# gargatik/Seamless-Through-Breaking-Rethinking-Image-Stitching-for-Optimal-Alignment

Hardware: AMD Instinct MI355X
Metric: stitched image-pairs/s at 512x512 (higher is better)
Workload: dtype f32 (decoder contractions, PatchEmbed's third conv and the C = 128 block tails: exact 3xbf16 split of both operands, 6 products on the bf16 matrix cores, fp32 accumulate -- error vs fp64 0.83x the fp32 MFMA chain's; everything else fp32); 1 GPU; UDIS-D-shaped 512x512 pairs, batch=1, FlowHomoAdpater.forward(type=test_eval); launch=hipGraph replay, pairs_in_flight=3

## Files before the change

include/stitch_gfx950.h:

```cpp
#ifndef STITCH_GFX950_H
#define STITCH_GFX950_H
#include <stdint.h>
#ifdef __cplusplus
extern "C" {
#endif

typedef struct st_gemm_desc {
    const float* a;
    const float* w;
    float* c;
    const float* bias;
    const float* aux0;
    const float* aux1;
    const float* aux2;
    const float* scale_ptr;
    int32_t M, N, K;
    int32_t H, W, Cin, ldx;
    int32_t kh, kw, sh, sw, ph, pw, Ho, Wo;
    int32_t ldw, ldc, ld_aux0, ld_aux1, ld_aux2;
    int32_t aux0_row_div, aux0_row_mod;
    int32_t act;
    int32_t epi;
    float alpha;
    int32_t batch;
// ... 66 lines not shown
    const float* w1;
    const float* b1;
    const float* w2;
    const float* b2;
    const float* res;
    int32_t lda, ldo, ld_res, M, hidden, ln;
    float ln_eps;
    int32_t reserved;
    const float* wp;
    const float* bp;
    const float* res0;
    int32_t ld_res0, reserved1;
} st_mlp_desc;
int st_mlp128(const st_mlp_desc* desc, void* stream);
int st_abi_mlp_desc_size(void);
int st_mlp128_split3_image_bytes(int32_t hidden, int32_t with_proj, int64_t* bytes);
int st_mlp128_split3_pack(const float* w1, const float* b1, const float* w2, const float* wp, const float* bp, int32_t hidden, void* image,
                          int64_t image_bytes, void* stream);
int st_mlp128_split3(const st_mlp_desc* desc, const void* image, int64_t image_bytes, void* stream);
int st_rowlin128_split3_image_bytes(int32_t N, int64_t* bytes);
int st_rowlin128_split3_pack(const float* w, const float* b, int32_t N, void* image, int64_t image_bytes, void* stream);
int st_rowlin128_split3(const float* a, int32_t lda, float* out, int32_t ldo, int32_t M, int32_t N, int32_t ln, float ln_eps, const void* image,
                        int64_t image_bytes, const float* aux, int32_t ld_aux, int32_t row_div, void* stream);

int st_corr_volume(const float* f1, const float* f2, float* vol, int32_t B, int32_t N1, int32_t N2,
                   int32_t C, void* stream);
int st_corr_volume_both(const float* f1, const float* f2, float* vol12, float* vol21, int32_t B, int32_t N, int32_t C,
                        void* stream);
int st_corr_volume_both_plan(int32_t B, int32_t N, int32_t C, int32_t aligned16);

int st_layernorm(const float* x, int32_t ldx, const float* w, const float* b, float* out, int32_t ldo,
                 int32_t rows, int32_t C, float eps, void* stream);
int st_softmax_rows(float* x, int32_t ld, int32_t rows, int32_t C, void* stream);
int st_l2norm_rows(const float* x, float* out, int32_t rows, int32_t C, void* stream);
int st_maxpool_nhwc(const float* x, float* out, int32_t B, int32_t H, int32_t W, int32_t C, int32_t k,
                    int32_t s, int32_t p, void* stream);
int st_dwconv3x3_residual(const float* x, const float* w, const float* bias, float* out, int32_t B,
                          int32_t H, int32_t W, int32_t C, void* stream);
int st_sine_pe(float* out, int32_t ld, int32_t rows, int32_t dim, const float* coords, int32_t ldc,
               int32_t Wg, int32_t ws, int32_t period, float cscale, float coff, int32_t accumulate,
               void* stream);
int st_attention_small(const float* q, int64_t q_bs, int64_t q_ts, const float* k, int64_t k_bs, int64_t k_ts,
                       const float* v, int64_t v_bs, int64_t v_ts, float* out, int64_t o_bs, int64_t o_ts,
                       int32_t B, int32_t heads, int32_t Nq, int32_t Nk, int32_t D, float scale, void* stream);
int st_attention_kvlds(const float* q, int64_t q_bs, int64_t q_ts, const float* k, int64_t k_bs, int64_t k_ts,
                       const float* v, int64_t v_bs, int64_t v_ts, float* out, int64_t o_bs, int64_t o_ts,
// ... 292 lines not shown
```

seamless-through-breaking-rethinking-image-stitching-for-optimal-alignment_amd/build.py:

```python
from __future__ import annotations

import os
import subprocess
import sys
from concurrent.futures import ThreadPoolExecutor

HERE = os.path.dirname(os.path.abspath(__file__))
CSRC = os.path.join(HERE, "csrc")
OUT = os.path.join(HERE, "libstitch_gfx950.so")
HIPCC = os.environ.get("HIPCC", "/opt/rocm/bin/hipcc")
SOURCES = {"gemm.hip": [], "gemm_split3.hip": [], "gemm_rows.hip": [], "nn.hip": [], "flowops.hip": [], "geom.hip": ["-ffp-contract=off"],
           "metrics.hip": ["-ffp-contract=off"], "operators.hip": [], "composition.hip": ["-ffp-contract=off"], "tps_pipeline.hip": ["-ffp-contract=off"], "patchembed.hip": [],
           "inpaint.hip": ["-ffp-contract=off"], "tps_other.hip": ["-ffp-contract=off"],
           "transref.hip": ["-ffp-contract=off"], "flow_splat.hip": ["-ffp-contract=off"], "jpeg.hip": [], "jpeg_dec.hip": [],
           "multiband.hip": ["-ffp-contract=off"], "exposure.hip": ["-ffp-contract=off"], "seam.hip": [], "seam_gc.hip": [], "crop.hip": [], "patchmatch.hip": [],
           "features.hip": ["-ffp-contract=off"], "dense_flow.hip": ["-ffp-contract=off"], "features_ms.hip": ["-ffp-contract=off"]}
COMMON = ["--offload-arch=gfx950", "-O3", "-std=c++17", "-fPIC", "-Wno-unused-result"]
COMMON += ["-Xclang", "-target-feature", "-Xclang", "-packed-fp32-ops"]
if os.environ.get("ST_EXACT_TRANSCENDENTALS", "0") == "1":
    COMMON.append("-DST_EXACT_TRANSCENDENTALS")


def compile_cmd(src, out, extra=()):
    return [HIPCC] + COMMON + SOURCES[src] + list(extra) + [os.path.join(CSRC, src), "-o", out]


def _stale(target, deps):
    if not os.path.exists(target):
        return True
    t = os.path.getmtime(target)
    return any(os.path.getmtime(d) > t for d in deps)


def build(force=False, verbose=False):
    hdrs = [os.path.join(CSRC, "common.h"), os.path.join(CSRC, "gemm_common.h"), os.path.join(CSRC, "gemm_split3.h"), os.path.join(CSRC, "mlp_split3.h"), os.path.join(CSRC, "tps_solve.h"), os.path.join(CSRC, "jpeg_dec_core.h"), os.path.join(CSRC, "jpeg_tables.h"), os.path.join(CSRC, "jpeg_huff_core.h"), os.path.join(CSRC, "jpeg_scan.h"), os.path.join(CSRC, "jpeg_rst_core.h"), os.path.join(CSRC, "features_common.h"), os.path.join(HERE, "..", "include", "stitch_gfx950.h")]
    objs, jobs = [], []
    os.makedirs(os.path.join(CSRC, "_obj"), exist_ok=True)
    for src in SOURCES:
        s = os.path.join(CSRC, src)
        o = os.path.join(CSRC, "_obj", src.replace(".hip", ".o"))
        objs.append(o)
        if force or _stale(o, [s] + hdrs):
            jobs.append(compile_cmd(src, o, ["-c"]))
    if jobs:
        def run(cmd):
            if verbose:
                print(" ".join(cmd), flush=True)
            r = subprocess.run(cmd, stderr=subprocess.PIPE, text=True)
            err = "".join(l for l in r.stderr.splitlines(True) if "'-packed-fp32-ops' is not a recognized feature for this target" not in l)
            if err:
                sys.stderr.write(err)
            if r.returncode:
                raise subprocess.CalledProcessError(r.returncode, cmd)
        with ThreadPoolExecutor(max_workers=4) as ex:
            list(ex.map(run, jobs))
    if jobs or _stale(OUT, objs):
        subprocess.check_call([HIPCC, "--offload-arch=gfx950", "-shared", "-fPIC", "-o", OUT] + objs)
    return OUT
# ... 5 lines not shown
```

seamless-through-breaking-rethinking-image-stitching-for-optimal-alignment_amd/csrc/gemm_rows.hip:

```cpp
#include "gemm_common.h"

static bool row_launch_begin(st_gemm_desc& od, int kernel, int tile, void* stream, const float* a, int lda, float* c, int ldc, const void* w, int M, int N,
                             int split3) {
    bool obs = st_observer_installed();
    if (obs) {
        od = Gemm(a, lda, (const float*)w, 128, c, ldc, M, N, 128).d;
        od.split3 = split3;
        obs = st_observe(&od, stream, 0);
    }
    st_plan_set(kernel, tile, 1, 1);
    return obs;
}

#define RC_NW 4
__global__ __launch_bounds__(256, 2) void rowchain128_kernel(const st_chain_desc d) {
    constexpr int NJ = 16, NW = RC_NW;
    extern __shared__ __attribute__((aligned(1024))) float smem[];
    float* ring = smem;
    const int tid = threadIdx.x, lane = tid & 63, wave = __builtin_amdgcn_readfirstlane(tid >> 6);
    const int li = lane & 31, lh = lane >> 5;
    const int nblk = (d.M + 31) >> 5;
    const int G = (int)gridDim.x;
    const int blk0 = (int)blockIdx.x * NW;
    const int rounds = blk0 < nblk ? (nblk - blk0 + G * NW - 1) / (G * NW) : 0;
// ... 456 lines not shown
}
extern "C" int st_rowlin128_split3(const float* a, int32_t lda, float* out, int32_t ldo, int32_t M, int32_t N, int32_t ln, float ln_eps, const void* image,
                                   int64_t image_bytes, const float* aux, int32_t ld_aux, int32_t row_div, void* stream) {
    if (aux && (ld_aux < N || (ld_aux & 3) || row_div < 1 || ((uintptr_t)aux & 15) || aux == out)) return ST_EINVAL;
    if (!a || !out || !image || M <= 0 || N < 32 || N > 4096 || (N & 31) || lda < 128 || ldo < N || (lda & 3) || (ldo & 3) || a == out) return ST_EINVAL;
    if ((((uintptr_t)a | (uintptr_t)out | (uintptr_t)image) & 15) || (int64_t)M * (lda > ldo ? lda : ldo) >= ((int64_t)1 << 40)) return ST_EINVAL;
    const int64_t need = (int64_t)(N / 32) * LS3_STAGE_B;
    if (image_bytes < need) return ST_EINVAL;
    const int nblk = (M + 31) / 32;
    int G = (nblk + 3) / 4;
    if (G > 512) G = 512;
    const size_t lds = (size_t)3 * LS3_STAGE_B;
    auto kern = aux ? rowlin128_split3_kernel<true> : rowlin128_split3_kernel<false>;
    (void)hipFuncSetAttribute((const void*)kern, hipFuncAttributeMaxDynamicSharedMemorySize, (int)lds);
    st_gemm_desc od;
    const bool obs = row_launch_begin(od, 10, 40, stream, a, lda, out, ldo, image, M, N, 1);
    hipLaunchKernelGGL(kern, dim3(G), dim3(256), lds, (hipStream_t)stream, a, (int)lda, out, (int)ldo, (int)M, (int)N, (int)ln, ln_eps,
                       (const unsigned char*)image, (unsigned)need, aux, (int)ld_aux, (int)(row_div > 0 ? row_div : 1));
    if (obs) st_observe(&od, stream, 1);
    ST_CHECK_LAUNCH();
    return ST_OK;
}

extern "C" int st_pe_tail_split3_image_bytes(int64_t* bytes) {
    if (!bytes) return ST_EINVAL;
    *bytes = PT3_IMAGE_B;
    return ST_OK;
}
extern "C" int st_pe_tail_split3_pack(const float* w1, int32_t ld1, const float* w2, void* image, int64_t image_bytes, void* stream) {
    if (!w1 || !w2 || !image || ld1 < 64 || ((uintptr_t)image & 15) || image_bytes < PT3_IMAGE_B) return ST_EINVAL;
    hipLaunchKernelGGL(pe_tail_split3_pack_kernel, dim3(3, 4), dim3(256), 0, (hipStream_t)stream, w1, (int)ld1, w2, (unsigned char*)image);
    ST_CHECK_LAUNCH();
    return ST_OK;
}
extern "C" int st_pe_tail_split3(const float* x, const float* tab, int32_t P, const void* image, int64_t image_bytes, const float* b2, const float* gamma,
                                 const float* beta, float eps, float* out, int32_t R, void* stream) {
    if (!x || !tab || !image || !b2 || !gamma || !beta || !out || R <= 0 || P <= 0 || image_bytes < PT3_IMAGE_B || x == out) return ST_EINVAL;
    if ((((uintptr_t)x | (uintptr_t)tab | (uintptr_t)image | (uintptr_t)out) & 15) || (int64_t)R * 128 >= ((int64_t)1 << 40)) return ST_EINVAL;
    const int nblk = (R + 31) / 32;
    int G = (nblk + 3) / 4;
    if (G > 256) G = 256;
    bool tabinv = false;
    for (int g = G; g >= (G > 8 ? G - G / 8 : 1); --g)
        if (((long)g * 128) % P == 0) { G = g; tabinv = true; break; }
    const size_t lds = (size_t)PT3_IMAGE_B + PT3_VEC_B;
    auto kern = tabinv ? pe_tail_split3_kernel<true> : pe_tail_split3_kernel<false>;
// ... 9 lines not shown
```

seamless-through-breaking-rethinking-image-stitching-for-optimal-alignment_amd/csrc/mlp_split3.h:

```cpp
#pragma once
#include "gemm_common.h"

#define MS3_W1_B 24576
#define MS3_W2_B 24576
#define MS3_BIAS_B 1024
#define MS3_STAGE_B (MS3_W1_B + MS3_W2_B + MS3_BIAS_B)
#define MS3_PIECES (MS3_STAGE_B / 1024)

typedef __bf16 bf16x2_t __attribute__((ext_vector_type(2)));
typedef float f32x2_t __attribute__((ext_vector_type(2)));

__device__ __forceinline__ unsigned ms3_pk(float a, float b) {
    const f32x2_t v = {a, b};
    return __builtin_bit_cast(unsigned, __builtin_convertvector(v, bf16x2_t));
}
__device__ __forceinline__ void ms3_split_pair(float x0, float x1, unsigned& h, unsigned& m, unsigned& l) {
    h = ms3_pk(x0, x1);
    const float r0 = x0 - __uint_as_float(h << 16), r1 = x1 - __uint_as_float(h & 0xffff0000u);
    m = ms3_pk(r0, r1);
    l = ms3_pk(r0 - __uint_as_float(m << 16), r1 - __uint_as_float(m & 0xffff0000u));
}

__global__ __launch_bounds__(256) void mlp_split3_pack_kernel(const float* __restrict__ w1, const float* __restrict__ b1, const float* __restrict__ w2,
                                                              const float* __restrict__ wp, const float* __restrict__ bp, int hidden,
// ... 445 lines not shown
                    MS3_SIX(acc, f, xp[0][ks], xp[1][ks], xp[2][ks])
#pragma unroll
                    for (int p = 0; p < 3; ++p) f[p] = fn[p];
                    __builtin_amdgcn_sched_barrier(0);
                }
                const float* bs = reinterpret_cast<const float*>(ws_ + MS3_W1_B);
                float4 v[4];
#pragma unroll
                for (int jj = 0; jj < 4; ++jj) {
                    const float4 bv = *reinterpret_cast<const float4*>(bs + 8 * jj + 4 * lh);
                    v[jj] = make_float4(acc[4 * jj] + bv.x, acc[4 * jj + 1] + bv.y, acc[4 * jj + 2] + bv.z, acc[4 * jj + 3] + bv.w);
                    if (AUX) { v[jj].x += ev[jj].x; v[jj].y += ev[jj].y; v[jj].z += ev[jj].z; v[jj].w += ev[jj].w; }
                }
                if (rok) {
#pragma unroll
                    for (int jj = 0; jj < 4; ++jj) *reinterpret_cast<float4*>(out + rowc * ldo + (c << 5) + 8 * jj + 4 * lh) = v[jj];
                }
            }
            g = g + 1 == 3 ? 0 : g + 1;
        }
    }
}


#define PT3_W1_B 12288
#define PT3_IMAGE_B (4 * PT3_W1_B + 4 * MS3_W2_B)
#define PT3_VEC_B 1536

__global__ __launch_bounds__(256) void pe_tail_split3_pack_kernel(const float* __restrict__ w1, const int ld1, const float* __restrict__ w2, unsigned char* __restrict__ image) {
    const int c = blockIdx.y, t = threadIdx.x;
    bf16x8 h, m, l;
    unsigned char* o;
    if (blockIdx.x == 0) {
        const int r = t >> 3, sl = t & 7, ks = sl >> 1, lh = sl & 1;
#pragma unroll
        for (int e = 0; e < 8; ++e) {
            __bf16 a0, a1, a2;
            st_split3(w1[(size_t)(32 * c + r) * ld1 + 16 * ks + 8 * (e >> 2) + 4 * lh + (e & 3)], a0, a1, a2);
            h[e] = a0; m[e] = a1; l[e] = a2;
        }
        o = image + c * PT3_W1_B + r * 128 + ((sl ^ ((r >> 1) & 7)) << 4);
        *reinterpret_cast<bf16x8*>(o) = h;
        *reinterpret_cast<bf16x8*>(o + 4096) = m;
        *reinterpret_cast<bf16x8*>(o + 8192) = l;
    } else {
        const int idx = (blockIdx.x - 1) * 256 + t, r = idx >> 2, sl = idx & 3, ks = sl >> 1, lh = sl & 1;
// ... 202 lines not shown
```

seamless-through-breaking-rethinking-image-stitching-for-optimal-alignment_amd/csrc/nn.hip:

```cpp
#include "common.h"
#include "../../include/stitch_gfx950.h"

__global__ __launch_bounds__(256) void layernorm_kernel(const float* __restrict__ x, int ldx, const float* __restrict__ w,
                                                        const float* __restrict__ b, float* __restrict__ out, int ldo,
                                                        int rows, int C, float eps) {
    const int row = (blockIdx.x * 256 + threadIdx.x) >> 6, lane = threadIdx.x & 63;
    if (row >= rows) return;
    const float* xr = x + (size_t)row * ldx;
    float v[16];
    float s = 0.f;
#pragma unroll
    for (int i = 0; i < 16; ++i) {
        const int c = lane + 64 * i;
        v[i] = c < C ? xr[c] : 0.f;
        s += v[i];
    }
    const float mean = wave_sum(s) / (float)C;
    float q = 0.f;
#pragma unroll
    for (int i = 0; i < 16; ++i) {
        const int c = lane + 64 * i;
        const float dlt = c < C ? v[i] - mean : 0.f;
        q += dlt * dlt;
    }
// ... 213 lines not shown
extern "C" int st_sine_pe(float* out, int32_t ld, int32_t rows, int32_t dim, const float* coords, int32_t ldc, int32_t Wg,
                          int32_t ws, int32_t period, float cscale, float coff, int32_t accumulate, void* stream) {
    if (!out || rows <= 0 || dim <= 0 || dim % 4 || ld < dim || (coords ? ldc < 2 : Wg <= 0) || ws < 0 || period < 0 || accumulate < 0) return ST_EINVAL;
    const size_t total = (size_t)rows * (dim / 4);
    hipLaunchKernelGGL(sine_pe_kernel, dim3((total + 255) / 256), dim3(256), 0, (hipStream_t)stream, out, ld, rows, dim,
                       coords, ldc, Wg, ws, period, cscale, coff, accumulate);
    ST_CHECK_LAUNCH();
    return ST_OK;
}

static bool al16(const void* p) { return ((uintptr_t)p & 15) == 0; }

template <int D>
__global__ __launch_bounds__(256) void attention_small_kernel(const float* __restrict__ q, long q_bs, long q_ts,
                                                              const float* __restrict__ k, long k_bs, long k_ts,
                                                              const float* __restrict__ v, long v_bs, long v_ts,
                                                              float* __restrict__ out, long o_bs, long o_ts, int B,
                                                              int heads, int Nq, int Nk, float scale) {
    const long idx = (long)blockIdx.x * 256 + threadIdx.x;
    if (idx >= (long)B * heads * Nq) return;
    const int iq = idx % Nq;
    const int h = (idx / Nq) % heads;
    const int b = idx / ((long)Nq * heads);
    float qr[D], acc[D];
    const float* qp = q + b * q_bs + iq * q_ts + h * D;
#pragma unroll
    for (int e = 0; e < D; e += 4) {
        const float4 t = *reinterpret_cast<const float4*>(qp + e);
        qr[e] = t.x * scale; qr[e + 1] = t.y * scale; qr[e + 2] = t.z * scale; qr[e + 3] = t.w * scale;
    }
    const float* kb = k + b * k_bs + h * D;
    const float* vb = v + b * v_bs + h * D;
    float mx = -INFINITY;
    for (int j = 0; j < Nk; ++j) {
        const float* kp = kb + j * k_ts;
        float s = 0.f;
#pragma unroll
        for (int e = 0; e < D; e += 4) {
            const float4 t = *reinterpret_cast<const float4*>(kp + e);
            s = fmaf(qr[e], t.x, s); s = fmaf(qr[e + 1], t.y, s); s = fmaf(qr[e + 2], t.z, s); s = fmaf(qr[e + 3], t.w, s);
        }
        mx = fmaxf(mx, s);
    }
#pragma unroll
    for (int e = 0; e < D; ++e) acc[e] = 0.f;
    float sum = 0.f;
    for (int j = 0; j < Nk; ++j) {
        const float* kp = kb + j * k_ts;
        float s = 0.f;
#pragma unroll
        for (int e = 0; e < D; e += 4) {
            const float4 t = *reinterpret_cast<const float4*>(kp + e);
            s = fmaf(qr[e], t.x, s); s = fmaf(qr[e + 1], t.y, s); s = fmaf(qr[e + 2], t.z, s); s = fmaf(qr[e + 3], t.w, s);
        }
        const float p = __expf(s - mx);
        sum += p;
        const float* vp = vb + j * v_ts;
#pragma unroll
        for (int e = 0; e < D; e += 4) {
            const float4 t = *reinterpret_cast<const float4*>(vp + e);
            acc[e] = fmaf(p, t.x, acc[e]); acc[e + 1] = fmaf(p, t.y, acc[e + 1]);
            acc[e + 2] = fmaf(p, t.z, acc[e + 2]); acc[e + 3] = fmaf(p, t.w, acc[e + 3]);
        }
    }
    const float inv = 1.0f / sum;
    float* op = out + b * o_bs + iq * o_ts + h * D;
#pragma unroll
    for (int e = 0; e < D; e += 4)
        *reinterpret_cast<float4*>(op + e) = make_float4(acc[e] * inv, acc[e + 1] * inv, acc[e + 2] * inv, acc[e + 3] * inv);
}

extern "C" int st_attention_small(const float* q, int64_t q_bs, int64_t q_ts, const float* k, int64_t k_bs, int64_t k_ts,
                                  const float* v, int64_t v_bs, int64_t v_ts, float* out, int64_t o_bs, int64_t o_ts,
                                  int32_t B, int32_t heads, int32_t Nq, int32_t Nk, int32_t D, float scale, void* stream) {
    if (!q || !k || !v || !out || B <= 0 || heads <= 0 || Nq <= 0 || Nk <= 0) return ST_EINVAL;
    if (!al16(q) || !al16(k) || !al16(v) || !al16(out) || ((q_bs | q_ts | k_bs | k_ts | v_bs | v_ts | o_bs | o_ts) & 3)) return ST_EINVAL;
    const long total = (long)B * heads * Nq;
    dim3 grid((total + 255) / 256), block(256);
    hipStream_t s = (hipStream_t)stream;
#define LAUNCH_AS(DD) hipLaunchKernelGGL(attention_small_kernel<DD>, grid, block, 0, s, q, q_bs, q_ts, k, k_bs, k_ts, v, \
                                         v_bs, v_ts, out, o_bs, o_ts, B, heads, Nq, Nk, scale)
    if (D == 8) LAUNCH_AS(8); else if (D == 16) LAUNCH_AS(16); else if (D == 32) LAUNCH_AS(32); else return ST_EINVAL;
#undef LAUNCH_AS
    ST_CHECK_LAUNCH();
    return ST_OK;
}

typedef float lp_f32x16 __attribute__((ext_vector_type(16)));

__global__ __launch_bounds__(256) void latent_pool_kernel(const float* __restrict__ scores, int ld_s, const float* __restrict__ tokens,
                                                          int ld_t, float* __restrict__ z, int P) {
    const size_t pix = blockIdx.x;
// ... 643 lines not shown
```

seamless-through-breaking-rethinking-image-stitching-for-optimal-alignment_amd/flowformer.py:

```python
from __future__ import annotations

import os

import torch
import torch.nn as nn

from . import ops
from .checkpoint import HP, ParamTree, flat_params, flow_spec
from .homography import pack_conv


SPLIT3 = os.environ.get("ST_SPLIT3", "1") != "0"


def _new(rows, cols, dev, zero=False):
    return (torch.zeros if zero else torch.empty)((rows, cols), device=dev, dtype=torch.float32)


def _planes_copy(p):
    return ops.Planes(p.rows, p.C, None, t=p.t.clone(), c0=p.c0, ncols=p.ncols)


def _keep(trace, **named):
    if trace is None:
# ... 105 lines not shown

        pk["fnet"] = twins("memory_encoder.feat_encoder.svt.")
        pk["cnet"] = twins("context_encoder.svt.")
        c = "memory_encoder.cost_perceiver_encoder."
        pe = dict(c0=conv(c + "patch_embed.proj.0"), c2=conv(c + "patch_embed.proj.2"), c4=conv(c + "patch_embed.proj.4"),
                  f0=conv(c + "patch_embed.ffn_with_coord.0"), f2=conv(c + "patch_embed.ffn_with_coord.2"),
                  norm=lin(c + "patch_embed.norm"))
        pe["c0_direct"] = (p[c + "patch_embed.proj.0.weight"].reshape(16, 36).t().contiguous(), pe["c0"][1])
        pe["embed11"] = [pe["c0_direct"][0], pe["c0_direct"][1], pe["c2"][0], pe["c2"][1], pe["c4"][0], pe["c4"][1],
                         pe["f0"][0], pe["f2"][0], pe["f2"][1], pe["norm"][0], pe["norm"][1]]
        if SPLIT3 and pe["c4"][0].is_cuda:
            pe["c4_s3"] = ops.split3_pack(pe["c4"][0])
            pe["tail_s3"] = ops.pe_tail_split3_pack(pe["f0"][0], pe["f2"][0])
        pk["pe"] = pe
        pk["latents"] = p[c + "latent_tokens"][0].contiguous()

        def attn_layer(name, fuse_qkv):
            d = dict(n1=lin(name + ".norm1"), n2=lin(name + ".norm2"), proj=lin(name + ".proj"), f0=lin(name + ".ffn.0"),
                     f3=lin(name + ".ffn.3"), q=lin(name + ".q"))
            if fuse_qkv:
                d["qkv"] = cat_lin([name + ".q", name + ".k", name + ".v"])
                d["qkv_ln"] = ops.fold_layernorm(*d["n1"], *d["qkv"])
                d["qkv_s3"] = lin_image(d["qkv_ln"])
            d["kv"] = cat_lin([name + ".k", name + ".v"])
            d["f0_ln"] = ops.fold_layernorm(*d["n2"], *d["f0"])
            d["mlp_s3"] = mlp_image(d["f0_ln"], d["f3"], d["proj"])
            d["mlp_s3_plain"] = mlp_image(d["f0_ln"], d["f3"], None)
            return d
        pk["xin"] = attn_layer(c + "input_layer", False)
        with torch.no_grad():
            L = pk["xin"]
            dev = L["proj"][0].device
            c64 = lambda t: t.detach().double().cpu()
            lat = c64(p[c + "latent_tokens"][0])
            qn = torch.nn.functional.layer_norm(lat, (lat.shape[1],), c64(L["n1"][0]), c64(L["n1"][1]), 1e-5)
            qv = qn @ c64(L["q"][0]).t() + c64(L["q"][1])
            Wk, Wv = c64(L["kv"][0][:128]), c64(L["kv"][0][128:])
            bv = c64(L["kv"][1][128:])
            nl_, hd = qv.shape[0], 16
            qp = torch.einsum("lhe,hec->lhc", qv.view(nl_, 8, hd), Wk.view(8, hd, 128)) * hd ** -0.5
            L["qfold"] = qp.reshape(nl_ * 8, 128).float().contiguous().to(dev)
            L["wv_heads"] = Wv.float().contiguous().to(dev)
            L["proj_b_fold"] = (c64(L["proj"][1]) + c64(L["proj"][0]) @ bv).float().contiguous().to(dev)
        pk["self"] = [attn_layer(c + f"encoder_layers.{i}", True) for i in range(HP["encoder_depth"])]
        vert = []
        for i in range(HP["encoder_depth"]):
# ... 176 lines not shown
            ops.latent_pool(S, tokens, z, M, P)
            ops.conv_gemm(z.view(M * nl, 8 * 128)[:, :128], L["wv_heads"][:16], att[:, :16], batch=8, bsa=128, bsw=16 * 128, bsc=16)
            proj_b = L["proj_b_fold"]
        else:
            qn = _new(nl, 128, dev)
            ops.layernorm(lat, L["n1"][0], L["n1"][1], qn, 1e-5)
            q = _new(nl, 128, dev)
            ops.conv_gemm(qn, L["q"][0], q, bias=L["q"][1])
            kv = _new(M * P, 256, dev)
            ops.conv_gemm(tokens, L["kv"][0], kv, bias=L["kv"][1])
            ops.attention_small(q, (0, 128), kv[:, :128], (P * 256, 256), kv[:, 128:], (P * 256, 256), att, (nl * 128, 128),
                                M, 8, nl, P, 16, 16 ** -0.5)
            proj_b = L["proj"][1]
        x1 = _new(M * nl, 128, dev)
        ops.conv_gemm(att, L["proj"][0], x1, bias=proj_b, aux0=lat, row_mod=nl)
        o = _new(M * nl, 128, dev)
        if L.get("mlp_s3_plain") is not None:
            return ops.mlp128(x1, o, L["f0_ln"][0], L["f0_ln"][1], L["f3"][0], L["f3"][1], ln_eps=1e-5, image=L["mlp_s3_plain"])
        return ops.linear_chain128(x1, o, [dict(w=L["f0_ln"][0], bias=L["f0_ln"][1], act="gelu", ln_eps=1e-5), dict(w=L["f3"][0], bias=L["f3"][1], res=0)])

    def _latent_self(self, L, x, M):
        dev = x.device
        nl = self._pk["latents"].shape[0]
        qkv = _new(M * nl, 384, dev)
        if L.get("qkv_s3") is not None:
            ops.rowlin128_split3(x, qkv, L["qkv_s3"], ln_eps=1e-5)
        else:
            ops.conv_gemm(x, L["qkv_ln"][0], qkv, bias=L["qkv_ln"][1], ln_eps=1e-5)
        att = _new(M * nl, 128, dev)
        ops.attention_small(qkv[:, :128], (nl * 384, 384), qkv[:, 128:256], (nl * 384, 384), qkv[:, 256:], (nl * 384, 384),
                            att, (nl * 128, 128), M, 8, nl, nl, 16, 16 ** -0.5)
        o = _new(M * nl, 128, dev)
        if L.get("mlp_s3") is not None:
            return ops.mlp128(att, o, L["f0_ln"][0], L["f0_ln"][1], L["f3"][0], L["f3"][1], ln_eps=1e-5, proj=(L["proj"][0], L["proj"][1], x), image=L["mlp_s3"])
        return ops.linear_chain128(att, o, [dict(w=L["proj"][0], bias=L["proj"][1], res=x),
                                            dict(w=L["f0_ln"][0], bias=L["f0_ln"][1], act="gelu", ln_eps=1e-5),
                                            dict(w=L["f3"][0], bias=L["f3"][1], res=1)])

    def _vertical(self, V, x, ctx, B, H1, W1, nl, extra_res=None):
        dev = x.device
        N = H1 * W1
        R = B * N * nl
        C, Cc = 128, 64
        Cq = C + Cc
        y = _new(R, C, dev)
        z = _new(B * N, Cq, dev)
        ops.conv_gemm(ctx, V["lctx"][0], z[:, C:], bias=V["lctx"][1])
        ops.sine_pe(z, Cq, Wg=W1, ws=7, period=N, accumulate=C)
        T = _new(B * N, 3 * C, dev)
        ops.conv_gemm(z, V["ltab"][0], T, bias=V["ltab"][1])
        qkv = _new(R, 3 * C, dev)
        if V.get("lqkv_s3") is not None:
            ops.rowlin128_split3(x, qkv, V["lqkv_s3"], ln_eps=1e-5, aux=T, row_div=nl)
        else:
# ... 226 lines not shown
```

seamless-through-breaking-rethinking-image-stitching-for-optimal-alignment_amd/ops.py:

```python
from __future__ import annotations

import ctypes as C
import warnings

import torch

from ._lib import ChainDesc, GemmDesc, JpegDecParams, JpegEncParams, MlpDesc, check, lib
from .jpeg_probe import JpegInfo, probe as _jpeg_probe
from ._lib import StitchError as StitchErrorBase

ACT = dict(none=0, relu=1, gelu=2, sigmoid=3, tanh=4, lrelu=5)
EPI = dict(store=0, add=1, mul=2, gru=3, axpy=4, zr=5)

assert lib.st_abi_gemm_desc_size() == C.sizeof(GemmDesc), "st_gemm_desc ABI mismatch between header and binding"
assert lib.st_abi_chain_desc_size() == C.sizeof(ChainDesc), "st_chain_desc ABI mismatch between header and binding"
assert lib.st_abi_mlp_desc_size() == C.sizeof(MlpDesc), "st_mlp_desc ABI mismatch between header and binding"
assert lib.st_abi_jpeg_dec_params_size() == C.sizeof(JpegDecParams), "st_jpeg_dec_params ABI mismatch between header and binding"
assert lib.st_abi_jpeg_enc_params_size() == C.sizeof(JpegEncParams), "st_jpeg_enc_params ABI mismatch between header and binding"


def _stream():
    return C.c_void_p(torch.cuda.current_stream().cuda_stream)


# ... 222 lines not shown
    return out


def rowlin128_split3_pack(w, b):
    N = w.shape[0]
    assert w.shape == (N, 128) and w.is_contiguous() and (b is None or b.shape == (N,))
    nb = C.c_int64(0)
    check(lib.st_rowlin128_split3_image_bytes(N, C.byref(nb)), "st_rowlin128_split3_image_bytes")
    img = torch.empty(nb.value, dtype=torch.uint8, device=w.device)
    check(lib.st_rowlin128_split3_pack(_p(w), _p(b), N, C.c_void_p(img.data_ptr()), nb.value, _stream()), "st_rowlin128_split3_pack")
    return img


def rowlin128_split3(a, out, image, ln_eps=None, aux=None, row_div=1):
    assert a.shape[1] == 128 and out.shape[0] == a.shape[0] and out.shape[1] % 32 == 0
    if aux is not None:
        assert aux.shape[1] == out.shape[1] and aux.shape[0] * row_div >= a.shape[0]
    check(lib.st_rowlin128_split3(_p(a), _ld(a), _p(out), _ld(out), a.shape[0], out.shape[1], 1 if ln_eps is not None else 0,
                                  float(ln_eps or 0.0), C.c_void_p(image.data_ptr()), image.numel(), _p(aux), _ld(aux) if aux is not None else 0, row_div,
                                  _stream()), "st_rowlin128_split3")
    return out


def mlp128_split3_pack(w1, b1, w2, proj=None):
    hidden = w1.shape[0]
    assert w1.shape == (hidden, 128) and w2.shape == (128, hidden) and w1.is_contiguous() and w2.is_contiguous() and b1.shape == (hidden,)
    nb = C.c_int64(0)
    check(lib.st_mlp128_split3_image_bytes(hidden, 1 if proj is not None else 0, C.byref(nb)), "st_mlp128_split3_image_bytes")
    img = torch.empty(nb.value, dtype=torch.uint8, device=w1.device)
    wp, bp = proj if proj is not None else (None, None)
    if wp is not None:
        assert wp.shape == (128, 128) and wp.is_contiguous()
    check(lib.st_mlp128_split3_pack(_p(w1), _p(b1), _p(w2), _p(wp) if wp is not None else None, _p(bp) if bp is not None else None, hidden,
                                    C.c_void_p(img.data_ptr()), nb.value, _stream()), "st_mlp128_split3_pack")
    return img


def mlp128(a, out, w1, b1, w2, b2, ln_eps=None, res=None, proj=None, image=None):
    hidden = w1.shape[0]
    assert w1.shape == (hidden, 128) and w2.shape == (128, hidden) and w1.is_contiguous() and w2.is_contiguous()
    assert b1.shape == (hidden,) and b2.shape == (128,) and a.shape[1] == 128 and out.shape == a.shape
    d = MlpDesc()
    d.a, d.out, d.lda, d.ldo, d.M, d.hidden = a.data_ptr(), out.data_ptr(), _ld(a), _ld(out), a.shape[0], hidden
    d.w1, d.b1, d.w2, d.b2 = w1.data_ptr(), b1.data_ptr(), w2.data_ptr(), b2.data_ptr()
    d.ln, d.ln_eps = (1, float(ln_eps)) if ln_eps is not None else (0, 0.0)
    if res is not None:
# ... 1635 lines not shown
```

Baseline: 93.00 pairs/s.

## Fuse latent self-attention QKV projection and attention into one split3 kernel

Adds a kernel that applies layernorm, runs the QKV projection on the split-bf16 matrix cores, and performs the 8-latent, 8-head attention in LDS per wave, writing only the attention output. This removes the intermediate QKV buffer round trip through global memory and one kernel launch per latent self-attention layer. The attention inner loop is factored into a shared device helper, which the existing small-attention kernel now also uses. The fused path applies only when split3 weights exist and there are 8 latents; otherwise the old two-kernel path runs.

```diff
diff --git a/include/stitch_gfx950.h b/include/stitch_gfx950.h
--- a/include/stitch_gfx950.h
+++ b/include/stitch_gfx950.h
@@ -112,6 +112,10 @@
 int st_rowlin128_split3_pack(const float* w, const float* b, int32_t N, void* image, int64_t image_bytes, void* stream);
 int st_rowlin128_split3(const float* a, int32_t lda, float* out, int32_t ldo, int32_t M, int32_t N, int32_t ln, float ln_eps, const void* image,
                         int64_t image_bytes, const float* aux, int32_t ld_aux, int32_t row_div, void* stream);
+int st_latent_self_attn_split3_image_bytes(int64_t* bytes);
+int st_latent_self_attn_split3_pack(const float* w, const float* b, void* image, int64_t image_bytes, void* stream);
+int st_latent_self_attn_split3(const float* a, int32_t lda, float* out, int32_t ldo, int32_t M, int32_t ln, float ln_eps, float scale,
+                               const void* image, int64_t image_bytes, void* stream);
 
 int st_corr_volume(const float* f1, const float* f2, float* vol, int32_t B, int32_t N1, int32_t N2,
                    int32_t C, void* stream);
diff --git a/seamless-through-breaking-rethinking-image-stitching-for-optimal-alignment_amd/build.py b/seamless-through-breaking-rethinking-image-stitching-for-optimal-alignment_amd/build.py
--- a/seamless-through-breaking-rethinking-image-stitching-for-optimal-alignment_amd/build.py
+++ b/seamless-through-breaking-rethinking-image-stitching-for-optimal-alignment_amd/build.py
@@ -33,7 +33,7 @@
 
 
 def build(force=False, verbose=False):
-    hdrs = [os.path.join(CSRC, "common.h"), os.path.join(CSRC, "gemm_common.h"), os.path.join(CSRC, "gemm_split3.h"), os.path.join(CSRC, "mlp_split3.h"), os.path.join(CSRC, "tps_solve.h"), os.path.join(CSRC, "jpeg_dec_core.h"), os.path.join(CSRC, "jpeg_tables.h"), os.path.join(CSRC, "jpeg_huff_core.h"), os.path.join(CSRC, "jpeg_scan.h"), os.path.join(CSRC, "jpeg_rst_core.h"), os.path.join(CSRC, "features_common.h"), os.path.join(HERE, "..", "include", "stitch_gfx950.h")]
+    hdrs = [os.path.join(CSRC, "common.h"), os.path.join(CSRC, "gemm_common.h"), os.path.join(CSRC, "gemm_split3.h"), os.path.join(CSRC, "mlp_split3.h"), os.path.join(CSRC, "attn_small.h"),os.path.join(CSRC, "tps_solve.h"), os.path.join(CSRC, "jpeg_dec_core.h"), os.path.join(CSRC, "jpeg_tables.h"), os.path.join(CSRC, "jpeg_huff_core.h"), os.path.join(CSRC, "jpeg_scan.h"), os.path.join(CSRC, "jpeg_rst_core.h"), os.path.join(CSRC, "features_common.h"), os.path.join(HERE, "..", "include", "stitch_gfx950.h")]
     objs, jobs = [], []
     os.makedirs(os.path.join(CSRC, "_obj"), exist_ok=True)
     for src in SOURCES:
diff --git a/seamless-through-breaking-rethinking-image-stitching-for-optimal-alignment_amd/csrc/attn_small.h b/seamless-through-breaking-rethinking-image-stitching-for-optimal-alignment_amd/csrc/attn_small.h
--- /dev/null
+++ b/seamless-through-breaking-rethinking-image-stitching-for-optimal-alignment_amd/csrc/attn_small.h
@@ -0,0 +1,40 @@
+#pragma once
+
+template <int D, class KF, class VF>
+__device__ __forceinline__ void st_attn_small_row(const float (&q)[D], const float scale, const int Nk, KF kf, VF vf, float (&o)[D]) {
+    float qr[D], acc[D];
+#pragma unroll
+    for (int e = 0; e < D; ++e) qr[e] = q[e] * scale;
+    float mx = -INFINITY;
+    for (int j = 0; j < Nk; ++j) {
+        float s = 0.f;
+#pragma unroll
+        for (int e = 0; e < D; e += 4) {
+            const float4 t = kf(j, e);
+            s = fmaf(qr[e], t.x, s); s = fmaf(qr[e + 1], t.y, s); s = fmaf(qr[e + 2], t.z, s); s = fmaf(qr[e + 3], t.w, s);
+        }
+        mx = fmaxf(mx, s);
+    }
+#pragma unroll
+    for (int e = 0; e < D; ++e) acc[e] = 0.f;
+    float sum = 0.f;
+    for (int j = 0; j < Nk; ++j) {
+        float s = 0.f;
+#pragma unroll
+        for (int e = 0; e < D; e += 4) {
+            const float4 t = kf(j, e);
+            s = fmaf(qr[e], t.x, s); s = fmaf(qr[e + 1], t.y, s); s = fmaf(qr[e + 2], t.z, s); s = fmaf(qr[e + 3], t.w, s);
+        }
+        const float p = __expf(s - mx);
+        sum += p;
+#pragma unroll
+        for (int e = 0; e < D; e += 4) {
+            const float4 t = vf(j, e);
+            acc[e] = fmaf(p, t.x, acc[e]); acc[e + 1] = fmaf(p, t.y, acc[e + 1]);
+            acc[e + 2] = fmaf(p, t.z, acc[e + 2]); acc[e + 3] = fmaf(p, t.w, acc[e + 3]);
+        }
+    }
+    const float inv = 1.0f / sum;
+#pragma unroll
+    for (int e = 0; e < D; ++e) o[e] = acc[e] * inv;
+}
diff --git a/seamless-through-breaking-rethinking-image-stitching-for-optimal-alignment_amd/csrc/gemm_rows.hip b/seamless-through-breaking-rethinking-image-stitching-for-optimal-alignment_amd/csrc/gemm_rows.hip
--- a/seamless-through-breaking-rethinking-image-stitching-for-optimal-alignment_amd/csrc/gemm_rows.hip
+++ b/seamless-through-breaking-rethinking-image-stitching-for-optimal-alignment_amd/csrc/gemm_rows.hip
@@ -502,6 +502,36 @@
     return ST_OK;
 }
 
+extern "C" int st_latent_self_attn_split3_image_bytes(int64_t* bytes) {
+    if (!bytes) return ST_EINVAL;
+    *bytes = LA3_IMAGE_B;
+    return ST_OK;
+}
+extern "C" int st_latent_self_attn_split3_pack(const float* w, const float* b, void* image, int64_t image_bytes, void* stream) {
+    if (!w || !image || ((uintptr_t)image & 15) || image_bytes != LA3_IMAGE_B) return ST_EINVAL;
+    hipLaunchKernelGGL(latent_self_attn_split3_pack_kernel, dim3(3, LA3_STEPS), dim3(256), 0, (hipStream_t)stream, w, b, (unsigned char*)image);
+    ST_CHECK_LAUNCH();
+    return ST_OK;
+}
+extern "C" int st_latent_self_attn_split3(const float* a, int32_t lda, float* out, int32_t ldo, int32_t M, int32_t ln, float ln_eps, float scale,
+                                          const void* image, int64_t image_bytes, void* stream) {
+    if (!a || !out || !image || M <= 0 || (M & 7) || lda < 128 || ldo < 128 || (lda & 3) || (ldo & 3) || a == out) return ST_EINVAL;
+    if ((((uintptr_t)a | (uintptr_t)out | (uintptr_t)image) & 15) || (int64_t)M * (lda > ldo ? lda : ldo) >= ((int64_t)1 << 40)) return ST_EINVAL;
+    if (image_bytes != LA3_IMAGE_B) return ST_EINVAL;
+    const int nblk = (M + 31) / 32;
+    int G = (nblk + 3) / 4;
+    if (G > 512) G = 512;
+    const size_t lds = (size_t)LA3_LDS_B;
+    (void)hipFuncSetAttribute((const void*)latent_self_attn_split3_kernel, hipFuncAttributeMaxDynamicSharedMemorySize, (int)lds);
+    st_gemm_desc od;
+    const bool obs = row_launch_begin(od, 12, 42, stream, a, lda, out, ldo, image, M, 384, 1);
+    hipLaunchKernelGGL(latent_self_attn_split3_kernel, dim3(G), dim3(256), lds, (hipStream_t)stream, a, (int)lda, out, (int)ldo, (int)M, (int)ln, ln_eps,
+                       scale, (const unsigned char*)image);
+    if (obs) st_observe(&od, stream, 1);
+    ST_CHECK_LAUNCH();
+    return ST_OK;
+}
+
 extern "C" int st_pe_tail_split3_image_bytes(int64_t* bytes) {
     if (!bytes) return ST_EINVAL;
     *bytes = PT3_IMAGE_B;
diff --git a/seamless-through-breaking-rethinking-image-stitching-for-optimal-alignment_amd/csrc/mlp_split3.h b/seamless-through-breaking-rethinking-image-stitching-for-optimal-alignment_amd/csrc/mlp_split3.h
--- a/seamless-through-breaking-rethinking-image-stitching-for-optimal-alignment_amd/csrc/mlp_split3.h
+++ b/seamless-through-breaking-rethinking-image-stitching-for-optimal-alignment_amd/csrc/mlp_split3.h
@@ -1,5 +1,6 @@
 #pragma once
 #include "gemm_common.h"
+#include "attn_small.h"
 
 #define MS3_W1_B 24576
 #define MS3_W2_B 24576
@@ -491,6 +492,185 @@
     }
 }
 
+#define LA3_STAGE_B MS3_W1_B
+#define LA3_STEPS 12
+#define LA3_BIAS_OFF (LA3_STEPS * LA3_STAGE_B)
+#define LA3_IMAGE_B (LA3_BIAS_OFF + 384 * 4)
+#define LA3_SLAB_B 8192
+#define LA3_LDS_B (2 * LA3_STAGE_B + 4 * LA3_SLAB_B)
+
+__global__ __launch_bounds__(256) void latent_self_attn_split3_pack_kernel(const float* __restrict__ w, const float* __restrict__ b, unsigned char* __restrict__ image) {
+    const int s = blockIdx.y, t = threadIdx.x;
+    const int f0 = (s % 3) * 128 + (s / 3) * 32;
+    if (blockIdx.x < 2) {
+        const int idx = blockIdx.x * 256 + t, r = idx >> 4, sl = idx & 15, ks = sl >> 1, lh = sl & 1;
+        const int feat = 16 * ((r >> 2) & 1) + 4 * (r >> 3) + (r & 3);
+        const float* W = w + (size_t)(f0 + feat) * 128;
+        bf16x8 h, m, l;
+#pragma unroll
+        for (int e = 0; e < 8; ++e) {
+            __bf16 a0, a1, a2;
+            st_split3(W[16 * ks + 8 * (e >> 2) + 4 * lh + (e & 3)], a0, a1, a2);
+            h[e] = a0; m[e] = a1; l[e] = a2;
+        }
+        unsigned char* o = image + (size_t)s * LA3_STAGE_B + r * 256 + ((sl ^ (r & 15)) << 4);
+        *reinterpret_cast<bf16x8*>(o) = h;
+        *reinterpret_cast<bf16x8*>(o + 8192) = m;
+        *reinterpret_cast<bf16x8*>(o + 16384) = l;
+    } else if (t < 32) {
+        reinterpret_cast<float*>(image + LA3_BIAS_OFF)[32 * s + t] = b ? b[f0 + t] : 0.f;
+    }
+}
+
+__global__ __launch_bounds__(256, 2) void latent_self_attn_split3_kernel(const float* __restrict__ a, const int lda, float* __restrict__ out, const int ldo, const int M,
+                                                                         const int ln, const float ln_eps, const float scale, const unsigned char* __restrict__ image) {
+    extern __shared__ __attribute__((aligned(1024))) unsigned char sm3[];
+    const int tid = threadIdx.x, lane = tid & 63, wave = __builtin_amdgcn_readfirstlane(tid >> 6);
+    const int li = lane & 31, lh = lane >> 5;
+    const int nblk = (M + 31) >> 5;
+    const int G = (int)gridDim.x;
+    const int blk0 = (int)blockIdx.x * 4;
+    const int rounds = blk0 < nblk ? (nblk - blk0 + G * 4 - 1) / (G * 4) : 0;
+    const int total = rounds * LA3_STEPS;
+    if (total == 0) return;
+    const unsigned lds0 = (unsigned)(size_t)(__attribute__((address_space(3))) unsigned char*)sm3;
+    const i32x4 rsd = make_rsrc(image, (unsigned)LA3_BIAS_OFF);
+    const unsigned vlin = (unsigned)lane << 4;
+    int s_dma = 0, g_dma = 0, q_dma = 0;
+#pragma clang diagnostic push
+#pragma clang diagnostic ignored "-Winline-asm"
+    auto dma_step = [&]() {
+        const unsigned dst = lds0 + (unsigned)(g_dma * LA3_STAGE_B), src = (unsigned)(s_dma * LA3_STAGE_B), o = (unsigned)wave * 6144u;
+        asm volatile("s_mov_b32 m0, %0\n\ts_nop 0\n\t"
+                     "buffer_load_dwordx4 %1, %2, %3 offen lds\n\t"
+                     "buffer_load_dwordx4 %1, %2, %3 offen offset:1024 lds\n\t"
+                     "buffer_load_dwordx4 %1, %2, %3 offen offset:2048 lds\n\t"
+                     "buffer_load_dwordx4 %1, %2, %3 offen offset:3072 lds"
+                     : : "s"(dst + o), "v"(vlin), "s"(rsd), "s"(src + o) : "memory", "m0");
+        asm volatile("s_mov_b32 m0, %0\n\ts_nop 0\n\t"
+                     "buffer_load_dwordx4 %1, %2, %3 offen lds\n\t"
+                     "buffer_load_dwordx4 %1, %2, %3 offen offset:1024 lds"
+                     : : "s"(dst + o + 4096u), "v"(vlin), "s"(rsd), "s"(src + o + 4096u) : "memory", "m0");
+        ++q_dma;
+        s_dma = s_dma + 1 == LA3_STEPS ? 0 : s_dma + 1;
+        g_dma ^= 1;
+    };
+#pragma clang diagnostic pop
+    dma_step();
+    int fo1[8];
+#pragma unroll
+    for (int ks = 0; ks < 8; ++ks) fo1[ks] = li * 256 + (((2 * ks + lh) ^ (li & 15)) << 4);
+    unsigned char* const slab = sm3 + 2 * LA3_STAGE_B + wave * LA3_SLAB_B;
+    const int sg = 4 * lh + (li >> 3), sgx = 2 * sg;
+    const int own = sg * 512, lr4 = 4 * (li & 7);
+    const float* const bias = reinterpret_cast<const float*>(image + LA3_BIAS_OFF) + 16 * lh;
+    int g = 0, step = 0;
+    for (int rd = 0; rd < rounds; ++rd) {
+        const int blk = blk0 + wave + rd * G * 4;
+        const bool active = blk < nblk;
+        const int row = blk * 32 + li;
+        const bool rok = active && row < M;
+        const size_t rowc = (size_t)(rok ? row : M - 1);
+        u32x4 xp[3][8];
+        if (active) {
+            float4 x[16];
+#pragma unroll
+            for (int j = 0; j < 16; ++j) x[j] = *reinterpret_cast<const float4*>(a + rowc * lda + 8 * j + 4 * lh);
+            if (ln) {
+                float s = 0.f;
+#pragma unroll
+                for (int j = 0; j < 16; ++j) s += (x[j].x + x[j].y) + (x[j].z + x[j].w);
+                s += __shfl_xor(s, 32, 64);
+                const float mean = s * (1.0f / 128.0f);
+                float v = 0.f;
+#pragma unroll
+                for (int j = 0; j < 16; ++j) {
+                    x[j].x -= mean; x[j].y -= mean; x[j].z -= mean; x[j].w -= mean;
+                    v += (x[j].x * x[j].x + x[j].y * x[j].y) + (x[j].z * x[j].z + x[j].w * x[j].w);
+                }
+                v += __shfl_xor(v, 32, 64);
+                const float rstd = 1.0f / sqrtf(v * (1.0f / 128.0f) + ln_eps);
+#pragma unroll
+                for (int j = 0; j < 16; ++j) { x[j].x *= rstd; x[j].y *= rstd; x[j].z *= rstd; x[j].w *= rstd; }
+            }
+#pragma unroll
+            for (int j = 0; j < 16; ++j) {
+                unsigned h0, m0, l0, h1, m1, l1;
+                ms3_split_pair(x[j].x, x[j].y, h0, m0, l0);
+                ms3_split_pair(x[j].z, x[j].w, h1, m1, l1);
+                xp[0][j >> 1][2 * (j & 1)] = h0; xp[0][j >> 1][2 * (j & 1) + 1] = h1;
+                xp[1][j >> 1][2 * (j & 1)] = m0; xp[1][j >> 1][2 * (j & 1) + 1] = m1;
+                xp[2][j >> 1][2 * (j & 1)] = l0; xp[2][j >> 1][2 * (j & 1) + 1] = l1;
+            }
+        }
+        __builtin_amdgcn_sched_barrier(0);
+        auto chunk = [&](const bool stores, float (&val)[16]) {
+            if (stores && active) asm volatile("s_waitcnt vmcnt(4)" ::: "memory");
+            else asm volatile("s_waitcnt vmcnt(0)" ::: "memory");
+            __syncthreads();
+            if (q_dma < total) dma_step();
+            if (active) {
+                const unsigned char* ws_ = sm3 + g * LA3_STAGE_B;
+                float4 bv[4];
+#pragma unroll
+                for (int jj = 0; jj < 4; ++jj) bv[jj] = *reinterpret_cast<const float4*>(bias + 32 * step + 4 * jj);
+                f32x16 acc;
+#pragma unroll
+                for (int r = 0; r < 16; ++r) acc[r] = 0.f;
+                u32x4 f[3], fn[3];
+#pragma unroll
+                for (int p = 0; p < 3; ++p) f[p] = *reinterpret_cast<const u32x4*>(ws_ + p * 8192 + fo1[0]);
+#pragma unroll
+                for (int ks = 0; ks < 8; ++ks) {
+                    const int kn = ks + 1 < 8 ? ks + 1 : ks;
+#pragma unroll
+                    for (int p = 0; p < 3; ++p) fn[p] = *reinterpret_cast<const u32x4*>(ws_ + p * 8192 + fo1[kn]);
+                    MS3_SIX(acc, f, xp[0][ks], xp[1][ks], xp[2][ks])
+#pragma unroll
+                    for (int p = 0; p < 3; ++p) f[p] = fn[p];
+                    __builtin_amdgcn_sched_barrier(0);
+                }
+#pragma unroll
+                for (int jj = 0; jj < 4; ++jj) {
+                    val[4 * jj] = acc[4 * jj] + bv[jj].x; val[4 * jj + 1] = acc[4 * jj + 1] + bv[jj].y;
+                    val[4 * jj + 2] = acc[4 * jj + 2] + bv[jj].z; val[4 * jj + 3] = acc[4 * jj + 3] + bv[jj].w;
+                }
+            }
+            g ^= 1;
+            step = step + 1 == LA3_STEPS ? 0 : step + 1;
+        };
+        auto to_slab = [&](const int off, const float (&val)[16]) {
+#pragma unroll
+            for (int u = 0; u < 4; ++u)
+                *reinterpret_cast<float4*>(slab + off + own + (((lr4 + u) ^ sgx) << 4)) = make_float4(val[4 * u], val[4 * u + 1], val[4 * u + 2], val[4 * u + 3]);
+        };
+#pragma unroll 1
+        for (int c = 0; c < 4; ++c) {
+            float qv[16], kv[16], ov[16];
+            chunk(c > 0, qv);
+            chunk(false, kv);
+            if (active) to_slab(0, kv);
+            chunk(false, kv);
+            if (active) {
+                to_slab(4096, kv);
+                __builtin_amdgcn_fence(__ATOMIC_RELEASE, "wavefront");
+                __builtin_amdgcn_wave_barrier();
+                __builtin_amdgcn_fence(__ATOMIC_ACQUIRE, "wavefront");
+                st_attn_small_row<16>(qv, scale, 8,
+                                      [&](int j, int e) { return *reinterpret_cast<const float4*>(slab + own + (((4 * j + (e >> 2)) ^ sgx) << 4)); },
+                                      [&](int j, int e) { return *reinterpret_cast<const float4*>(slab + 4096 + own + (((4 * j + (e >> 2)) ^ sgx) << 4)); }, ov);
+                __builtin_amdgcn_fence(__ATOMIC_RELEASE, "wavefront");
+                __builtin_amdgcn_wave_barrier();
+                if (rok) {
+                    float* op = out + rowc * ldo + 32 * c + 16 * lh;
+#pragma unroll
+                    for (int u = 0; u < 4; ++u) *reinterpret_cast<float4*>(op + 4 * u) = make_float4(ov[4 * u], ov[4 * u + 1], ov[4 * u + 2], ov[4 * u + 3]);
+                }
+            }
+        }
+    }
+}
+
 
 #define PT3_W1_B 12288
 #define PT3_IMAGE_B (4 * PT3_W1_B + 4 * MS3_W2_B)
diff --git a/seamless-through-breaking-rethinking-image-stitching-for-optimal-alignment_amd/csrc/nn.hip b/seamless-through-breaking-rethinking-image-stitching-for-optimal-alignment_amd/csrc/nn.hip
--- a/seamless-through-breaking-rethinking-image-stitching-for-optimal-alignment_amd/csrc/nn.hip
+++ b/seamless-through-breaking-rethinking-image-stitching-for-optimal-alignment_amd/csrc/nn.hip
@@ -1,4 +1,5 @@
 #include "common.h"
+#include "attn_small.h"
 #include "../../include/stitch_gfx950.h"
 
 __global__ __launch_bounds__(256) void layernorm_kernel(const float* __restrict__ x, int ldx, const float* __restrict__ w,
@@ -259,52 +260,20 @@
     const int iq = idx % Nq;
     const int h = (idx / Nq) % heads;
     const int b = idx / ((long)Nq * heads);
-    float qr[D], acc[D];
+    float qv[D], ov[D];
     const float* qp = q + b * q_bs + iq * q_ts + h * D;
 #pragma unroll
     for (int e = 0; e < D; e += 4) {
         const float4 t = *reinterpret_cast<const float4*>(qp + e);
-        qr[e] = t.x * scale; qr[e + 1] = t.y * scale; qr[e + 2] = t.z * scale; qr[e + 3] = t.w * scale;
+        qv[e] = t.x; qv[e + 1] = t.y; qv[e + 2] = t.z; qv[e + 3] = t.w;
     }
     const float* kb = k + b * k_bs + h * D;
     const float* vb = v + b * v_bs + h * D;
-    float mx = -INFINITY;
-    for (int j = 0; j < Nk; ++j) {
-        const float* kp = kb + j * k_ts;
-        float s = 0.f;
-#pragma unroll
-        for (int e = 0; e < D; e += 4) {
-            const float4 t = *reinterpret_cast<const float4*>(kp + e);
-            s = fmaf(qr[e], t.x, s); s = fmaf(qr[e + 1], t.y, s); s = fmaf(qr[e + 2], t.z, s); s = fmaf(qr[e + 3], t.w, s);
-        }
-        mx = fmaxf(mx, s);
-    }
-#pragma unroll
-    for (int e = 0; e < D; ++e) acc[e] = 0.f;
-    float sum = 0.f;
-    for (int j = 0; j < Nk; ++j) {
-        const float* kp = kb + j * k_ts;
-        float s = 0.f;
-#pragma unroll
-        for (int e = 0; e < D; e += 4) {
-            const float4 t = *reinterpret_cast<const float4*>(kp + e);
-            s = fmaf(qr[e], t.x, s); s = fmaf(qr[e + 1], t.y, s); s = fmaf(qr[e + 2], t.z, s); s = fmaf(qr[e + 3], t.w, s);
-        }
-        const float p = __expf(s - mx);
-        sum += p;
-        const float* vp = vb + j * v_ts;
-#pragma unroll
-        for (int e = 0; e < D; e += 4) {
-            const float4 t = *reinterpret_cast<const float4*>(vp + e);
-            acc[e] = fmaf(p, t.x, acc[e]); acc[e + 1] = fmaf(p, t.y, acc[e + 1]);
-            acc[e + 2] = fmaf(p, t.z, acc[e + 2]); acc[e + 3] = fmaf(p, t.w, acc[e + 3]);
-        }
-    }
-    const float inv = 1.0f / sum;
+    st_attn_small_row<D>(qv, scale, Nk, [&](int j, int e) { return *reinterpret_cast<const float4*>(kb + j * k_ts + e); },
+                         [&](int j, int e) { return *reinterpret_cast<const float4*>(vb + j * v_ts + e); }, ov);
     float* op = out + b * o_bs + iq * o_ts + h * D;
 #pragma unroll
-    for (int e = 0; e < D; e += 4)
-        *reinterpret_cast<float4*>(op + e) = make_float4(acc[e] * inv, acc[e + 1] * inv, acc[e + 2] * inv, acc[e + 3] * inv);
+    for (int e = 0; e < D; e += 4) *reinterpret_cast<float4*>(op + e) = make_float4(ov[e], ov[e + 1], ov[e + 2], ov[e + 3]);
 }
 
 extern "C" int st_attention_small(const float* q, int64_t q_bs, int64_t q_ts, const float* k, int64_t k_bs, int64_t k_ts,
diff --git a/seamless-through-breaking-rethinking-image-stitching-for-optimal-alignment_amd/flowformer.py b/seamless-through-breaking-rethinking-image-stitching-for-optimal-alignment_amd/flowformer.py
--- a/seamless-through-breaking-rethinking-image-stitching-for-optimal-alignment_amd/flowformer.py
+++ b/seamless-through-breaking-rethinking-image-stitching-for-optimal-alignment_amd/flowformer.py
@@ -151,6 +151,7 @@
                 d["qkv"] = cat_lin([name + ".q", name + ".k", name + ".v"])
                 d["qkv_ln"] = ops.fold_layernorm(*d["n1"], *d["qkv"])
                 d["qkv_s3"] = lin_image(d["qkv_ln"])
+                d["attn_s3"] = ops.latent_self_attn_split3_pack(*d["qkv_ln"]) if d["qkv_s3"] is not None else None
             d["kv"] = cat_lin([name + ".k", name + ".v"])
             d["f0_ln"] = ops.fold_layernorm(*d["n2"], *d["f0"])
             d["mlp_s3"] = mlp_image(d["f0_ln"], d["f3"], d["proj"])
@@ -373,14 +374,17 @@
     def _latent_self(self, L, x, M):
         dev = x.device
         nl = self._pk["latents"].shape[0]
-        qkv = _new(M * nl, 384, dev)
-        if L.get("qkv_s3") is not None:
-            ops.rowlin128_split3(x, qkv, L["qkv_s3"], ln_eps=1e-5)
-        else:
-            ops.conv_gemm(x, L["qkv_ln"][0], qkv, bias=L["qkv_ln"][1], ln_eps=1e-5)
         att = _new(M * nl, 128, dev)
-        ops.attention_small(qkv[:, :128], (nl * 384, 384), qkv[:, 128:256], (nl * 384, 384), qkv[:, 256:], (nl * 384, 384),
-                            att, (nl * 128, 128), M, 8, nl, nl, 16, 16 ** -0.5)
+        if L.get("attn_s3") is not None and nl == 8:
+            ops.latent_self_attn_split3(x, att, L["attn_s3"], ln_eps=1e-5, scale=16 ** -0.5)
+        else:
+            qkv = _new(M * nl, 384, dev)
+            if L.get("qkv_s3") is not None:
+                ops.rowlin128_split3(x, qkv, L["qkv_s3"], ln_eps=1e-5)
+            else:
+                ops.conv_gemm(x, L["qkv_ln"][0], qkv, bias=L["qkv_ln"][1], ln_eps=1e-5)
+            ops.attention_small(qkv[:, :128], (nl * 384, 384), qkv[:, 128:256], (nl * 384, 384), qkv[:, 256:], (nl * 384, 384),
+                                att, (nl * 128, 128), M, 8, nl, nl, 16, 16 ** -0.5)
         o = _new(M * nl, 128, dev)
         if L.get("mlp_s3") is not None:
             return ops.mlp128(att, o, L["f0_ln"][0], L["f0_ln"][1], L["f3"][0], L["f3"][1], ln_eps=1e-5, proj=(L["proj"][0], L["proj"][1], x), image=L["mlp_s3"])
diff --git a/seamless-through-breaking-rethinking-image-stitching-for-optimal-alignment_amd/ops.py b/seamless-through-breaking-rethinking-image-stitching-for-optimal-alignment_amd/ops.py
--- a/seamless-through-breaking-rethinking-image-stitching-for-optimal-alignment_amd/ops.py
+++ b/seamless-through-breaking-rethinking-image-stitching-for-optimal-alignment_amd/ops.py
@@ -268,6 +268,22 @@
     return out
 
 
+def latent_self_attn_split3_pack(w, b):
+    assert w.shape == (384, 128) and w.is_contiguous() and (b is None or b.shape == (384,))
+    nb = C.c_int64(0)
+    check(lib.st_latent_self_attn_split3_image_bytes(C.byref(nb)), "st_latent_self_attn_split3_image_bytes")
+    img = torch.empty(nb.value, dtype=torch.uint8, device=w.device)
+    check(lib.st_latent_self_attn_split3_pack(_p(w), _p(b), C.c_void_p(img.data_ptr()), nb.value, _stream()), "st_latent_self_attn_split3_pack")
+    return img
+
+
+def latent_self_attn_split3(a, out, image, ln_eps=None, scale=16 ** -0.5):
+    assert a.shape[1] == 128 and out.shape == (a.shape[0], 128)
+    check(lib.st_latent_self_attn_split3(_p(a), _ld(a), _p(out), _ld(out), a.shape[0], 1 if ln_eps is not None else 0, float(ln_eps or 0.0), float(scale),
+                                         C.c_void_p(image.data_ptr()), image.numel(), _stream()), "st_latent_self_attn_split3")
+    return out
+
+
 def mlp128_split3_pack(w1, b1, w2, proj=None):
     hidden = w1.shape[0]
     assert w1.shape == (hidden, 128) and w2.shape == (128, hidden) and w1.is_contiguous() and w2.is_contiguous() and b1.shape == (hidden,)
```

After: 93.95 pairs/s (median of 6 runs). +1.0%, better.
